# xandercai/JSPSR

Measured on AMD Instinct MI355X. Metric: Mpixels/sec fwd+bwd, JSPSR x8 on 512^2 DEM tiles, higher is better.
Workload: dtype bf16; 1 GPU; jspsr_r8_img_msk (image+mask guided, 43.87M params), 8 x 512x512 tiles per GPU, train step (fwd + L1/L2/Sobel loss + bwd + grad all-reduce + AdamW); storage policy: bf16 activations / gradients / MFMA operands, fp32 accumulation, BatchNorm statistics, master weights and optimizer, and the generator head (affinity logits + offsets) kept as fp32 planes; tiles_per_gpu=8, tile=512, global_tiles=8, parallelism=dp1, step_mode=eager

## Files before the change

### include/jspsr_hip.h

```cpp
#ifndef JSPSR_HIP_H
#define JSPSR_HIP_H

#include <stddef.h>
#include <stdint.h>

#ifdef __cplusplus
extern "C" {
#endif

#define JSPSR_OK 0
#define JSPSR_EINVAL (-1)
#define JSPSR_EALIGN (-2)

typedef void* jspsr_stream_t;

int jspsr_abi_version(void);
long long jspsr_launch_count(const char* what);
int jspsr_conv_dynamic_queue(int on);
const char* jspsr_last_error(void);

int jspsr_prop_forward_f32(const float* dem, const float* weight, const float* offset,
                           int offset_channels, const float* wk, const float* b0, float scale,
                           float* out, int B, int H, int W, jspsr_stream_t stream);

size_t jspsr_prop_backward_workspace_bytes(int B, int H, int W);

int jspsr_prop_backward_f32(const float* grad_out, const float* dem, const float* weight,
                            const float* offset, int offset_channels, const float* wk,
                            float* grad_weight, float* grad_offset, float* grad_wk,
                            float* grad_b0, void* workspace, int B, int H, int W,
                            jspsr_stream_t stream);

int jspsr_prop_backward_fold_f32(const void* workspace, int B, int H, int W, float* grad_wk, float* grad_b0,
                                 jspsr_stream_t stream);

int jspsr_prop_step_forward_f32(const float* dem, const float* weight, const float* offset, int offset_channels,
                                const float* wk, const float* b0, float scale, int normalize, float* out,
                                int B, int H, int W, jspsr_stream_t stream);
size_t jspsr_prop_step_backward_workspace_bytes(int B, int H, int W);
int jspsr_prop_step_backward_f32(const float* grad_out, const float* dem, const float* weight, const float* offset,
                                 int offset_channels, const float* wk, float scale, int normalize, int accumulate,
// ... 46 lines not shown
int jspsr_conv_head1_backward(int dtype, const float* dy, const void* x, int x_cstride, int x_coff, int C, const float* w,
                              void* dx, int dx_cstride, int dx_coff, float* dw, float* db, void* workspace, int B, int H,
                              int W, jspsr_stream_t stream);

#define JSPSR_F32 0
#define JSPSR_BF16 1

int jspsr_pack_weight(int dtype, const float* w, void* packed, int O, int I, int KH, int KW,
                      int mode, int c_pad, jspsr_stream_t stream);

typedef struct jspsr_pack_desc {
  const float* w;
  void* out;
  long long start;
  long long total;
  int O, I, KH, KW;
  int mode;
  int c_pad;
  int dtype;
  int reserved;
} jspsr_pack_desc;
int jspsr_pack_chunk(void);
int jspsr_pack_weights_multi(const jspsr_pack_desc* descs, int n, long long total_blocks, jspsr_stream_t stream);

int jspsr_conv2d_stats_rows(int B, int OH, int OW);
int jspsr_conv2d_in_affine_ok(int dtype, int Cin, int KH, int KW, int stride);
int jspsr_conv2d_forward(int dtype, const void* in, const void* wpack, const float* bias, void* out,
                         int B, int IH, int IW, int Cin, int in_cstride, int in_coff, int Cout,
                         int out_cstride, int out_coff, int KH, int KW, int stride, int pad, int relu,
                         float* stats, const float* scale, const void* addend, int add_cstride,
                         const float* in_affine, int in_relu, jspsr_stream_t stream);
int jspsr_conv2d_forward_scaled(int dtype, const void* in, const void* wpack, const float* bias, void* out,
                                int B, int IH, int IW, int Cin, int in_cstride, int in_coff, int Cout,
                                int out_cstride, int out_coff, int KH, int KW, int stride, int pad, int relu,
                                float* stats, const float* scale, const void* addend, int add_cstride,
                                const float* in_scale, int in_scale_bstride, jspsr_stream_t stream);

int jspsr_conv2d_dgrad_reduce_ok(int dtype, int B, int IH, int IW, int Cg, int Cin, int KH, int KW, int stride, int pad);
int jspsr_conv2d_dgrad(int dtype, const void* gout, const void* wpack_t, const float* bias, void* gin,
                       int B, int OH, int OW, int Cg, int g_cstride, int g_coff, int IH, int IW,
                       int Cin, int in_cstride, int in_coff, int KH, int KW, int stride, int pad,
                       int relu, const void* addend, int add_cstride, const float* scale,
                       const void* red_x, int red_cstride, const float* red_par, float* red_out, jspsr_stream_t stream);

size_t jspsr_conv2d_wgrad_workspace_bytes(int dtype, int B, int OH, int OW, int Cg, int Cx, int KH, int KW);
int jspsr_conv2d_wgrad_x_affine_ok(int dtype, int B, int OH, int OW, int Cg, int Cx, int KH, int KW, int stride, int pad);
// ... 176 lines not shown
```

### jspsr_amd/_lib.py

```python
from __future__ import annotations

import ctypes
import os
import subprocess
import threading

_HERE = os.path.dirname(os.path.abspath(__file__))
SO_PATH = os.environ.get("JSPSR_LAB_LIB") or os.path.join(_HERE, "lib", "libjspsr_hip.so")
CSRC = os.path.join(_HERE, "csrc")
ABI_VERSION = 25

_lock = threading.Lock()
_lib = None

c_p = ctypes.c_void_p
c_i = ctypes.c_int
c_f = ctypes.c_float
c_ll = ctypes.c_longlong

SIGNATURES = {
    "jspsr_abi_version": (c_i, []),
    "jspsr_launch_count": (c_ll, [ctypes.c_char_p]),
    "jspsr_conv_dynamic_queue": (c_i, [c_i]),
    "jspsr_last_error": (ctypes.c_char_p, []),
    "jspsr_prop_forward_f32": (c_i, [c_p, c_p, c_p, c_i, c_p, c_p, c_f, c_p, c_i, c_i, c_i, c_p]),
    "jspsr_prop_backward_workspace_bytes": (ctypes.c_size_t, [c_i, c_i, c_i]),
    "jspsr_prop_backward_f32": (c_i, [c_p] * 4 + [c_i] + [c_p] * 6 + [c_i, c_i, c_i, c_p]),
    "jspsr_prop_backward_fold_f32": (c_i, [c_p, c_i, c_i, c_i, c_p, c_p, c_p]),
    "jspsr_prop_step_forward_f32": (c_i, [c_p, c_p, c_p, c_i, c_p, c_p, c_f, c_i, c_p, c_i, c_i, c_i, c_p]),
    "jspsr_prop_step_backward_workspace_bytes": (ctypes.c_size_t, [c_i, c_i, c_i]),
    "jspsr_prop_step_backward_f32": (c_i, [c_p] * 4 + [c_i, c_p, c_f, c_i, c_i] + [c_p] * 6 + [c_i, c_i, c_i, c_p]),
    "jspsr_prop_head_forward": (c_i, [c_i, c_p, c_p, c_p, c_p, c_f, c_p, c_i, c_i, c_i, c_p]),
    "jspsr_prop_head_backward_workspace_bytes": (ctypes.c_size_t, [c_i, c_i, c_i]),
    "jspsr_prop_head_backward": (c_i, [c_i] + [c_p] * 8 + [c_i, c_i, c_i, c_p]),
    "jspsr_prop_logits_forward_f32": (c_i, [c_p, c_p, c_p, c_p, c_f, c_p, c_i, c_i, c_i, c_p]),
    "jspsr_prop_logits_backward_f32": (c_i, [c_p] * 8 + [c_i, c_i, c_i, c_p]),
    "jspsr_head_ok": (c_i, [c_i] * 5),
    "jspsr_head_forward": (c_i, [c_i, c_p, c_i, c_i, c_i, c_p, c_p, c_p, c_i, c_i, c_i, c_p]),
    "jspsr_head_backward_workspace_bytes": (ctypes.c_size_t, [c_i, c_i, c_i]),
    "jspsr_head_backward": (c_i, [c_i, c_p, c_p, c_i, c_p, c_i, c_i, c_p, c_p, c_p, c_i, c_i, c_i, c_p]),
    "jspsr_conv_head1_forward": (c_i, [c_i, c_p, c_i, c_i, c_i, c_p, c_p, c_p, c_i, c_i, c_i, c_p]),
    "jspsr_conv_head1_workspace_bytes": (ctypes.c_size_t, [c_i, c_i, c_i, c_i]),
    "jspsr_conv_head1_backward": (c_i, [c_i, c_p, c_p, c_i, c_i, c_i, c_p, c_p, c_i, c_i, c_p, c_p, c_p, c_i, c_i, c_i, c_p]),
    "jspsr_pack_weight": (c_i, [c_i, c_p, c_p] + [c_i] * 6 + [c_p]),
    "jspsr_pack_chunk": (c_i, []),
    "jspsr_pack_weights_multi": (c_i, [c_p, c_i, c_ll, c_p]),
    "jspsr_conv2d_stats_rows": (c_i, [c_i, c_i, c_i]),
    "jspsr_conv2d_in_affine_ok": (c_i, [c_i] * 5),
    "jspsr_conv2d_forward": (c_i, [c_i] + [c_p] * 4 + [c_i] * 14 + [c_p, c_p, c_p, c_i, c_p, c_i, c_p]),
    "jspsr_conv2d_forward_scaled": (c_i, [c_i] + [c_p] * 4 + [c_i] * 14 + [c_p, c_p, c_p, c_i, c_p, c_i, c_p]),
    "jspsr_bn_fold": (c_i, [c_p, c_p, c_p, c_p, c_f, c_f, c_i, c_p, c_p, c_p]),
    "jspsr_conv2d_dgrad_reduce_ok": (c_i, [c_i] * 10),
    "jspsr_conv2d_dgrad": (c_i, [c_i] + [c_p] * 4 + [c_i] * 16 + [c_p, c_i, c_p, c_p, c_i, c_p, c_p, c_p]),
    "jspsr_conv2d_wgrad_workspace_bytes": (ctypes.c_size_t, [c_i] * 8),
    "jspsr_conv2d_wgrad_x_affine_ok": (c_i, [c_i] * 10),
    "jspsr_conv2d_wgrad": (c_i, [c_i, c_p, c_i, c_i, c_i, c_p, c_i, c_i, c_i, c_p] + [c_i] * 12 + [c_p, c_i, c_p, c_p]),
    "jspsr_conv2d_wgrad_scaled": (c_i, [c_i, c_p, c_i, c_i, c_i, c_p, c_i, c_i, c_i, c_p] + [c_i] * 12 + [c_p, c_i, c_p, c_p]),
    "jspsr_reduce_workspace_bytes": (ctypes.c_size_t, [c_i, c_i, c_i]),
    "jspsr_bn_forward": (c_i, [c_i, c_p, c_i, c_i, c_p, c_i, c_i, c_p, c_i, c_i, c_p, c_p, c_p, c_p, c_f, c_f, c_i,
                               c_i, c_f, c_p, c_p, c_ll, c_i, c_p, c_i, c_p, c_p, c_p, c_p, c_p]),
    "jspsr_bn_mask_bytes": (ctypes.c_size_t, [c_i, c_ll, c_i]),
    "jspsr_bn_reduce_params": (c_i, [c_p, c_p, c_p, c_p, c_i, c_p, c_p]),
    "jspsr_bn_backward": (c_i, [c_i, c_p, c_i, c_i, c_p, c_i, c_i, c_p, c_i, c_i, c_p, c_p, c_p, c_p, c_i, c_i, c_f,
                                c_p, c_p, c_p, c_p, c_i, c_ll, c_i, c_p, c_p, c_i, c_p, c_p]),
    "jspsr_act_backward": (c_i, [c_i, c_p, c_i, c_i, c_p, c_i, c_i, c_p, c_i, c_p, c_ll, c_i, c_p, c_p]),
    "jspsr_gate_pool": (c_i, [c_i, c_p, c_i, c_ll, c_i, c_p, c_p, c_p, c_p, c_p]),
    "jspsr_gate_scale": (c_i, [c_i, c_p, c_p, c_p, c_i, c_ll, c_i, c_p]),
    "jspsr_gate_backward_reduce": (c_i, [c_i, c_p, c_p, c_p, c_i, c_ll, c_i, c_p, c_p]),
    "jspsr_gate_backward_apply": (c_i, [c_i, c_p, c_p, c_p, c_p, c_p, c_p, c_i, c_ll, c_i, c_p]),
# ... 108 lines not shown
```

### jspsr_amd/csrc/conv.hip

```cpp
#include "conv_igemm.h"

#include <cstdlib>
#include <type_traits>

namespace {

using namespace jspsr;

constexpr int NT = 256;
constexpr int NCH = 8;
template <typename T> struct Elem;
template <> struct Elem<float> { static constexpr int EPC = 4; };
template <> struct Elem<__bf16> { static constexpr int EPC = 8; };

template <typename T> struct Mma;
template <> struct Mma<float> {
  static constexpr int BLK = 32, ROWP = 144, NE = 16, SUB = NCH / 2, SUBB = 32;
  using acc_t = f32x16;
  static __device__ __forceinline__ int frag_row(int lane) { return lane & 31; }
  static __device__ __forceinline__ int frag_chunk(int lane) { return lane >> 5; }
  static __device__ __forceinline__ int acc_row(int lane, int e) { return (e & 3) + 8 * (e >> 2) + 4 * (lane >> 5); }
  static __device__ __forceinline__ int acc_col(int lane) { return lane & 31; }
};
template <> struct Mma<__bf16> {
// ... 1042 lines not shown
    const int mid = (lo + hi + 1) >> 1;
    if (descs[mid].start <= b) lo = mid; else hi = mid - 1;
  }
  const jspsr_pack_desc d = descs[lo];
  const long long l0 = (b - d.start) * PACK_CHUNK;
  const float* __restrict__ w = d.w;
#pragma unroll
  for (int k = 0; k < PACK_CHUNK / 256; ++k) {
    const long long l = l0 + k * 256 + threadIdx.x;
    if (l >= d.total) break;
    const int c = (int)(l % d.c_pad);
    long long r = l / d.c_pad;
    const int kx = (int)(r % d.KW); r /= d.KW;
    const int ky = (int)(r % d.KH); r /= d.KH;
    const int nn = (int)r;
    float v = 0.f;
    if (d.mode == 0) { if (c < d.I) v = w[(((size_t)nn * d.I + c) * d.KH + ky) * d.KW + kx]; }
    else             { if (c < d.O) v = w[(((size_t)c * d.I + nn) * d.KH + ky) * d.KW + kx]; }
    if (d.dtype == JSPSR_F32) static_cast<float*>(d.out)[l] = v;
    else static_cast<__bf16*>(d.out)[l] = (__bf16)v;
  }
}

}

extern "C" int jspsr_pack_weights_multi(const jspsr_pack_desc* descs, int n, long long total_blocks, jspsr_stream_t stream) {
  if (!descs || n <= 0 || total_blocks <= 0 || total_blocks > 0x7fffffffLL) return fail(JSPSR_EINVAL, "pack_weights_multi: bad arguments");
  hipLaunchKernelGGL(pack_weights_multi_kernel, dim3((unsigned)total_blocks), dim3(256), 0, static_cast<hipStream_t>(stream), descs, n);
  return check_launch("pack_weights_multi");
}

extern "C" int jspsr_pack_chunk(void) { return PACK_CHUNK; }

extern "C" int jspsr_pack_weight(int dtype, const float* w, void* packed, int O, int I, int KH, int KW,
                                 int mode, int c_pad, jspsr_stream_t stream) {
  if (!w || !packed || O <= 0 || I <= 0 || KH <= 0 || KW <= 0 || (mode != 0 && mode != 1))
    return fail(JSPSR_EINVAL, "pack_weight: bad arguments");
  const int C = mode == 0 ? I : O, N = mode == 0 ? O : I;
  if (c_pad < C) return fail(JSPSR_EINVAL, "pack_weight: c_pad %d < %d", c_pad, C);
  const long long total = (long long)N * KH * KW * c_pad;
  const int blocks = (int)((total + 255) / 256 < 4096 ? (total + 255) / 256 : 4096);
  hipStream_t s = static_cast<hipStream_t>(stream);
  if (dtype == JSPSR_F32)
    hipLaunchKernelGGL(pack_weight_kernel<float>, dim3(blocks), dim3(256), 0, s, w, static_cast<float*>(packed), O, I, KH, KW, mode, c_pad, total);
  else if (dtype == JSPSR_BF16)
    hipLaunchKernelGGL(pack_weight_kernel<__bf16>, dim3(blocks), dim3(256), 0, s, w, static_cast<__bf16*>(packed), O, I, KH, KW, mode, c_pad, total);
  else
    return fail(JSPSR_EINVAL, "pack_weight: bad dtype");
  return check_launch("pack_weight");
}

extern "C" int jspsr_conv2d_stats_rows(int B, int OH, int OW) {
  if (B <= 0 || OH <= 0 || OW <= 0) return 0;
  return B * ((OH + 7) / 8) * ((OW + 15) / 16);
}
// ... 128 lines not shown
```

### jspsr_amd/csrc/elementwise.hip

```cpp
#include "common.h"

#include <atomic>
#include <cstdlib>

namespace {

using namespace jspsr;

constexpr int TX = 64, TY = 4;

template <typename T> struct V;
template <> struct V<float> { static constexpr int N = 4; };
template <> struct V<__bf16> { static constexpr int N = 8; };

template <typename T, int N>
struct Pack { T v[N]; };

template <typename T>
__device__ __forceinline__ uint4 load_raw(const T* p) { return *reinterpret_cast<const uint4*>(p); }
template <typename T>
__device__ __forceinline__ void unpack(const uint4& raw, float (&f)[V<T>::N]) {
  if constexpr (sizeof(T) == 4) {
    f[0] = __uint_as_float(raw.x); f[1] = __uint_as_float(raw.y); f[2] = __uint_as_float(raw.z); f[3] = __uint_as_float(raw.w);
  } else {
// ... 686 lines not shown
                                void* mask_out, void* workspace, jspsr_stream_t stream) {
  if (int e = check_c(dtype, C, "bn_forward")) return e;
  if (!x || (!y && !affine_out) || !gamma || !beta || !save_mean || !save_invstd || !workspace || npix <= 0)
    return fail(JSPSR_EINVAL, "bn_forward: null pointer or empty tensor");
  if (res_affine && !res) return fail(JSPSR_EINVAL, "bn_forward: res_affine without a residual operand");
  if (mask_out && (!res || !relu || !y)) return fail(JSPSR_EINVAL, "bn_forward: mask_out needs an output with residual and ReLU");
  if (!training && (!running_mean || !running_var)) return fail(JSPSR_EINVAL, "bn_forward: eval mode needs running stats");
  const int vec = dtype == JSPSR_F32 ? 4 : 8;
  if (x_cs % vec || x_coff % vec || y_cs % vec || y_coff % vec || (res && (r_cs % vec || r_coff % vec)))
    return fail(JSPSR_EINVAL, "bn_forward: channel pitches/offsets must be multiples of %d", vec);
  hipStream_t s = static_cast<hipStream_t>(stream);
  float* ws = static_cast<float*>(workspace);
  float* scale = affine_out ? affine_out : ws;
  float* shift = affine_out ? affine_out + C : ws + C;
  float* partial = ws + 2 * C;
  int rows = 0;
  if (training && ext_partial) {
    if (ext_rows <= 0) return fail(JSPSR_EINVAL, "bn_forward: ext_rows must be positive");
    rows = ext_rows < 256 ? ext_rows : 256;
    if (ext_rows > 256) {
      hipLaunchKernelGGL(fold_rows_kernel, dim3(rows, (2 * C + 255) / 256), dim3(256), 0, s, ext_partial, ext_rows, 2 * C, rows, partial);
      if (int e = check_launch("bn_fold_rows")) return e;
    } else {
      (void)hipMemcpyAsync(partial, ext_partial, (size_t)ext_rows * 2 * C * sizeof(float), hipMemcpyDeviceToDevice, s);
    }
  } else if (training) {
    const RedGeom g = make_red(npix, 1, C, vec);
    rows = g.chunks;
    DISPATCH(dtype, hipLaunchKernelGGL(bn_stats_kernel<T>, red_grid(g, vec), dim3(TX, TY), 0, s,
                                       static_cast<const T*>(x), x_cs, x_coff, g, partial));
    if (int e = check_launch("bn_stats")) return e;
  }
  hipLaunchKernelGGL(bn_finalize_kernel, dim3((C + 3) / 4), dim3(256), 0, s, partial, rows, C, npix, gamma, beta,
                     running_mean, running_var, momentum, eps, training, save_mean, save_invstd, scale, shift);
  if (int e = check_launch("bn_finalize")) return e;
  if (!y) return JSPSR_OK;
  const RedGeom ga = make_red(npix, 1, C, vec);
#define BN_APPLY(R, M) DISPATCH(dtype, hipLaunchKernelGGL((bn_apply_kernel<T, R, M>), red_grid(ga, vec), dim3(TX, TY), 0, s,       \
                                     static_cast<const T*>(x), x_cs, x_coff, static_cast<const T*>(res), r_cs, r_coff,        \
                                     static_cast<T*>(y), y_cs, y_coff, scale, shift, res_affine, res_scale, relu,             \
                                     static_cast<unsigned char*>(mask_out), ga))
  if (mask_out) { BN_APPLY(true, true); } else if (res) { BN_APPLY(true, false); } else { BN_APPLY(false, false); }
#undef BN_APPLY
  return check_launch("bn_apply");
}

__global__ void bn_reduce_params_kernel(const float* __restrict__ gamma, const float* __restrict__ beta, const float* __restrict__ mean,
// ... 511 lines not shown
```

### jspsr_amd/csrc/wgrad.hip

```cpp
#include "conv_igemm.h"

#include <type_traits>

namespace {

using namespace jspsr;

constexpr int NT = 256;
using s16x4 = __attribute__((ext_vector_type(4))) short;

struct WgradGeom {
  int B, OH, OW;
  int Cg, g_cs, g_coff;
  int IH, IW;
  int Cx, x_cs, x_coff;
  int KH, KW, stride, pad;
  int Ktot;
  int m_per_split;
  long long M;
};

template <typename T> struct WT;
template <> struct WT<float> { static constexpr int EPC = 4, BKM = 32; };
template <> struct WT<__bf16> { static constexpr int EPC = 8, BKM = 64; };
// ... 502 lines not shown
      }
    red[zl][ex] = s;
    __syncthreads();
    if (zl == 0 && idx < total) {
      float t[4] = {0.f, 0.f, 0.f, 0.f};
#pragma unroll
      for (int q = 0; q < 8; ++q) {
        const float4 v = red[q][ex];
        t[0] += v.x; t[1] += v.y; t[2] += v.z; t[3] += v.w;
      }
#pragma unroll
      for (int j = 0; j < 4; ++j) {
        const long long i = idx + j;
        const int r = (int)(i / Ktot), k = (int)(i % Ktot);
        const int tap = k / Cx, c = k % Cx;
        if (c < C) {
          const size_t dst = ((size_t)r * C + c) * (KH * KW) + tap;
          dW[dst] = accumulate ? dW[dst] + t[j] : t[j];
        }
      }
    }
    __syncthreads();
  }
}

struct Plan {
  int bmc, splits, m_per_split;
};

template <typename T>
Plan make_plan(long long M, int Cg, int Ktot) {
  Plan p;
  p.bmc = Cg > 64 ? 128 : (Cg > 32 ? 64 : 32);
  const int BKM = WT<T>::BKM;
  const long long tiles = (long long)((Cg + p.bmc - 1) / p.bmc) * ((Ktot + 127) / 128);
  long long splits = (768 + tiles - 1) / tiles;
  const long long max_splits = (M + 4 * BKM - 1) / (4 * BKM);
  if (splits > max_splits) splits = max_splits;
  if (splits < 1) splits = 1;
  long long per = (M + splits - 1) / splits;
  per = (per + BKM - 1) / BKM * BKM;
  p.m_per_split = (int)per;
  p.splits = (int)((M + per - 1) / per);
  return p;
}

// ... 19 lines not shown
    const PatchPlan pp = make_patch_plan<T>(g.B, g.OH, g.OW, g.Cg, g.Cx);
    const long long img_g = (long long)g.OH * g.OW * g.g_cs * (long long)sizeof(T);
    const long long img_x = (long long)g.IH * g.IW * g.x_cs * (long long)sizeof(T);
    if (pp.ok && img_g < 0xF0000000LL && img_x < 0xF0000000LL) {
      PatchGeom q{};
      q.B = g.B; q.H = g.OH; q.W = g.OW;
      q.Cg = g.Cg; q.g_cs = g.g_cs; q.g_coff = g.g_coff;
      q.Cx = g.Cx; q.x_cs = g.x_cs; q.x_coff = g.x_coff;
      q.Ktot = g.Ktot; q.strips_x = g.OW / WP<T>::U;
      q.rows_per_blk = pp.rows_per_blk; q.row_blks = pp.row_blks;
      q.pairs_g = (g.Cg + 63) / 64; q.pairs_x = (g.Cx + 63) / 64;
      q.x_affine = x_affine; q.x_relu = x_relu; q.x_bstride = x_bstride; q.x_scale_only = x_scale_only;
      const long long nblk = (long long)pp.units * q.pairs_g * q.pairs_x;
      if (x_affine && x_scale_only)
        hipLaunchKernelGGL((wgrad_patch_kernel<T, 2>), dim3((unsigned)nblk), dim3(NT), 0, s, static_cast<const T*>(G),
                           static_cast<const T*>(X), ws, q);
      else if (x_affine)
        hipLaunchKernelGGL((wgrad_patch_kernel<T, 1>), dim3((unsigned)nblk), dim3(NT), 0, s, static_cast<const T*>(G),
                           static_cast<const T*>(X), ws, q);
      else
        hipLaunchKernelGGL((wgrad_patch_kernel<T, 0>), dim3((unsigned)nblk), dim3(NT), 0, s, static_cast<const T*>(G),
                           static_cast<const T*>(X), ws, q);
      if (int e = check_launch("conv2d_wgrad_patch")) return e;
      const long long total = (long long)R * g.Ktot;
      const int blocks = (int)((total + 127) / 128 < 4096 ? (total + 127) / 128 : 4096);
      hipLaunchKernelGGL(wgrad_reduce_kernel, dim3(blocks), dim3(256), 0, s, ws, dW, R, C, g.KH, g.KW, g.Cg, g.Cx,
                         pp.units, accumulate);
      return check_launch("conv2d_wgrad_reduce");
    }
  }
  if (x_affine) return fail(JSPSR_EINVAL, "conv2d_wgrad: x_affine needs the nine-tap kernel (3x3, stride 1, pad 1): ask jspsr_conv2d_wgrad_x_affine_ok first");
  const Plan p = make_plan<T>(g.M, g.Cg, g.Ktot);
  g.m_per_split = p.m_per_split;
  const long long g_slice = (long long)p.m_per_split * g.g_cs * (long long)sizeof(T);
  const long long imgs = p.m_per_split / ((long long)g.OH * g.OW) + 2;
  const long long x_span = imgs * g.IH * g.IW * (long long)g.x_cs * (long long)sizeof(T);
  if (g_slice >= 0xF0000000LL || (x_span >= 0xF0000000LL && (long long)g.B * g.IH * g.IW * g.x_cs * (long long)sizeof(T) >= 0xF0000000LL))
    return fail(JSPSR_EINVAL, "conv2d_wgrad: tensor slice exceeds the 32-bit offset range of one launch");
  int e;
  if (p.bmc == 128) e = launch_w<T, 128, 2, 2>(G, X, ws, g, p.splits, s);
  else if (p.bmc == 64) e = launch_w<T, 64, 2, 2>(G, X, ws, g, p.splits, s);
  else e = launch_w<T, 32, 1, 4>(G, X, ws, g, p.splits, s);
  if (e) return e;
  const long long total = (long long)R * g.Ktot;
  const int blocks = (int)((total + 127) / 128 < 4096 ? (total + 127) / 128 : 4096);
  hipLaunchKernelGGL(wgrad_reduce_kernel, dim3(blocks), dim3(256), 0, s, ws, dW, R, C, g.KH, g.KW, g.Cg, g.Cx,
                     p.splits, accumulate);
  return check_launch("conv2d_wgrad_reduce");
}

}

extern "C" size_t jspsr_conv2d_wgrad_workspace_bytes(int dtype, int B, int OH, int OW, int Cg, int Cx, int KH, int KW) {
  if (B <= 0 || OH <= 0 || OW <= 0 || Cg <= 0 || Cx <= 0 || KH <= 0 || KW <= 0) return 0;
  const long long M = (long long)B * OH * OW;
  const int Ktot = KH * KW * Cx;
  const Plan p = dtype == JSPSR_BF16 ? make_plan<__bf16>(M, Cg, Ktot) : make_plan<float>(M, Cg, Ktot);
  size_t splits = (size_t)p.splits;
  if (KH == 3 && KW == 3) {
    const PatchPlan pp = dtype == JSPSR_BF16 ? make_patch_plan<__bf16>(B, OH, OW, Cg, Cx) : make_patch_plan<float>(B, OH, OW, Cg, Cx);
    if (pp.ok && (size_t)pp.units > splits) splits = (size_t)pp.units;
  }
  return splits * Cg * Ktot * sizeof(float);
}

static int conv2d_wgrad_impl(int dtype, const void* G, int Cg, int g_cstride, int g_coff, const void* X, int Cx,
                             int x_cstride, int x_coff, float* dW, int R, int C, int B, int OH, int OW,
                             int IH, int IW, int KH, int KW, int stride, int pad, int accumulate,
                             const float* x_affine, int x_relu, int x_bstride, int x_scale_only, void* workspace,
                             jspsr_stream_t stream) {
  if (dtype != JSPSR_F32 && dtype != JSPSR_BF16) return fail(JSPSR_EINVAL, "conv2d_wgrad: bad dtype");
  if (x_affine && !aligned16(x_affine)) return fail(JSPSR_EALIGN, "conv2d_wgrad: x_affine must be 16-byte aligned");
  if (!G || !X || !dW || !workspace) return fail(JSPSR_EINVAL, "conv2d_wgrad: null pointer");
// ... 44 lines not shown
```

### jspsr_amd/graph.py

```python
from __future__ import annotations

import torch

from . import ops


class GraphedStep:

    def __init__(self, model, reducer, optimizer, criterion, inputs, target, warmup: int = 3):
        if reducer.world != 1:
            raise RuntimeError("GraphedStep: single-process steps only (a captured step holds no collective)")
        if not model.training:
            raise RuntimeError("GraphedStep captures a TRAINING step: call model.train() first")
        self.model, self.reducer, self.opt, self.criterion = model, reducer, optimizer, criterion
        self.inputs = [t.detach().clone() for t in inputs]
        self.target = target.detach().clone()
        optimizer.enable_device_hyper()
        if hasattr(criterion, "reset"):
            criterion.reset()
        import gc
        gc.collect()
        side = torch.cuda.Stream()
        side.wait_stream(torch.cuda.current_stream())
        with torch.cuda.stream(side):
            for _ in range(warmup):
                self._body()
            if hasattr(criterion, "reset"):
                criterion.reset()
        torch.cuda.current_stream().wait_stream(side)
        torch.cuda.synchronize()
        self.warmup_steps = warmup
        steps_before = optimizer.steps
        self.graph = torch.cuda.CUDAGraph()
        with torch.cuda.graph(self.graph, stream=side):
            self.loss = self._body()
        optimizer.steps = steps_before
        self.replays = 0

    def _body(self):
        self.reducer.zero_grad()
        loss = self.criterion(self.model(*self.inputs), self.target)["Total"]
        loss.backward()
        self.reducer.finish()
        self.opt.step()
        return loss

    def __call__(self, inputs=None, target=None):
        if inputs is not None:
            for dst, src in zip(self.inputs, inputs):
                dst.copy_(src, non_blocking=True)
        if target is not None:
            self.target.copy_(target, non_blocking=True)
        self.opt.steps += 1
        self.opt.upload_hyper()
        self.graph.replay()
        ops.invalidate_packed_weights()
        self.replays += 1
        return self.loss
```

### jspsr_amd/kernels.py

```python
from __future__ import annotations

import torch

from . import _lib

F32, BF16 = 0, 1


def _dt(t: torch.Tensor) -> int:
    if t.dtype == torch.float32:
        return F32
    if t.dtype == torch.bfloat16:
        return BF16
    raise TypeError(f"unsupported dtype {t.dtype}")


def epc(dtype: torch.dtype) -> int:
    return 4 if dtype == torch.float32 else 8


def _stream() -> int:
    return torch.cuda.current_stream().cuda_stream


# ... 9 lines not shown
        return False
    B, H, W, C = t.shape
    p = t.stride(2)
    if p < C or (H > 1 and t.stride(1) != W * p) or (B > 1 and t.stride(0) != H * W * p) or W == 1:
        return False
    return t.data_ptr() % 16 == 0 and (p * t.element_size()) % 16 == 0


def pitch(t: torch.Tensor) -> int:
    return t.shape[3] if t.is_contiguous() else t.stride(2)


def nhwc(t: torch.Tensor) -> torch.Tensor:
    return t if (t.is_contiguous() or is_slice(t)) else t.contiguous()


def _chk_s(t: torch.Tensor, name: str):
    if not t.is_cuda:
        raise RuntimeError(f"{name}: jspsr_amd kernels run on the GPU only (no CPU fallback)")
    if not (t.is_contiguous() or is_slice(t)):
        raise ValueError(f"{name}: expected a dense NHWC tensor or a channel slice of one")


def pack_weight(w: torch.Tensor, mode: int, c_pad: int, dtype: torch.dtype) -> torch.Tensor:
    _chk(w, "pack_weight")
    O, I, KH, KW = w.shape
    n = O if mode == 0 else I
    out = torch.empty((n, KH, KW, c_pad), dtype=dtype, device=w.device)
    lib = _lib.load()
    _lib.check(lib.jspsr_pack_weight(_dt(out), w.data_ptr(), out.data_ptr(), O, I, KH, KW, mode, c_pad, _stream()),
               "jspsr_pack_weight")
    return out


def fused_input_ok(dtype, B, OH, OW, Cin, Cout, KH, KW, stride, pad) -> bool:
    lib = _lib.load()
    dt = F32 if dtype == torch.float32 else BF16
    return bool(lib.jspsr_conv2d_in_affine_ok(dt, Cin, KH, KW, stride)) and \
        bool(lib.jspsr_conv2d_wgrad_x_affine_ok(dt, B, OH, OW, Cout, Cin, KH, KW, stride, pad))


def _chk_scale(t, B, C, name):
    if t.dtype != torch.float32 or not t.is_cuda or not t.is_contiguous() or tuple(t.shape) != (B, C):
        raise ValueError(f"{name}: expected a contiguous fp32 ({B}, {C}) tensor on the GPU, got {tuple(t.shape)} {t.dtype}")


def in_scale_ok(dtype, Cin, KH, KW, stride) -> bool:
    return bool(_lib.load().jspsr_conv2d_in_affine_ok(F32 if dtype == torch.float32 else BF16, Cin, KH, KW, stride))


def x_scale_ok(dtype, B, OH, OW, Cout, Cin, KH, KW, stride, pad) -> bool:
# ... 316 lines not shown
```

### jspsr_amd/ops.py

```python
from __future__ import annotations

import collections
import os
import weakref

import torch

from . import _lib
from . import kernels as K


def _stream() -> int:
    return torch.cuda.current_stream().cuda_stream


def _need_gpu(*ts):
    for t in ts:
        if not t.is_cuda:
            raise RuntimeError("jspsr_amd ops run on the GPU only (got a CPU tensor); there is no CPU fallback")
        if t.dtype != torch.float32:
            raise TypeError(f"expected float32, got {t.dtype}")


def prop_forward_raw(dem, weight, offset, w, b, scale, out):
# ... 393 lines not shown
        ws = torch.empty(max(lib.jspsr_prop_backward_workspace_bytes(B, H, W), 16), dtype=torch.uint8, device=dem.device)
        _lib.check(lib.jspsr_prop_logits_backward_f32(grad_out.data_ptr(), dem.data_ptr(), head.data_ptr(), w.data_ptr(),
                                                      ghead.data_ptr(), gw.data_ptr(), gb.data_ptr(), ws.data_ptr(), B, H, W,
                                                      _stream()), "jspsr_prop_logits_backward_f32")
        return None, ghead, gw, gb, None


def propagate_logits(dem, head, w, b, scale: float = 1.0):
    if dem.requires_grad:
        raise RuntimeError("propagate_logits: dem must be detached (no gradient with respect to the DEM is produced)")
    return _PropagateLogits.apply(dem, head, w, b, scale)




_weights_epoch = 0


def invalidate_packed_weights():
    global _weights_epoch
    _weights_epoch += 1


repack_after_step = os.environ.get("JSPSR_REPACK_ALL", "0") != "0"
_pack_registry = {}
_pack_table = None


def _packed(param, w, mode, c_pad, dtype):
    if not isinstance(param, torch.nn.Parameter):
        return K.pack_weight(w, mode, c_pad, dtype)
    cache = param.__dict__.setdefault("_jspsr_packs", {})
    key = (mode, c_pad, dtype, w.data_ptr())
    hit = cache.get(key)
    stamp = (param._version, _weights_epoch)
    if hit is not None and hit[1] == stamp:
        return hit[0]
    if len(cache) > 8:
        cache.clear()
    packed = K.pack_weight(w, mode, c_pad, dtype)
    cache[key] = (packed, stamp)
    if id(param) not in _pack_registry:
        _pack_registry[id(param)] = weakref.ref(param, lambda _, k=id(param): _pack_registry.pop(k, None))
    return packed


def repack_all():
    global _pack_table
    import numpy as np
    entries = []
    for ref in list(_pack_registry.values()):
        p = ref()
        if p is None or not p.is_cuda:
            continue
        for (mode, c_pad, dtype, ptr), (packed, _) in p.__dict__.get("_jspsr_packs", {}).items():
            if ptr == p.data_ptr() and p.dim() == 4 and p.is_contiguous():
                entries.append((p, mode, c_pad, dtype, packed))
    if not entries:
        return 0
    sig = tuple((p.data_ptr(), packed.data_ptr(), mode, c_pad) for p, mode, c_pad, _, packed in entries)
    if _pack_table is None or _pack_table[0] != sig:
        desc = np.zeros(len(entries), dtype=np.dtype([("w", "<u8"), ("out", "<u8"), ("start", "<i8"), ("total", "<i8"),
                                                      ("O", "<i4"), ("I", "<i4"), ("KH", "<i4"), ("KW", "<i4"), ("mode", "<i4"),
                                                      ("c_pad", "<i4"), ("dtype", "<i4"), ("reserved", "<i4")]))
        start, chunk = 0, _lib.load().jspsr_pack_chunk()
        for i, (p, mode, c_pad, dtype, packed) in enumerate(entries):
            O, I, KH, KW = p.shape
            total = packed.numel()
            desc[i] = (p.data_ptr(), packed.data_ptr(), start, total, O, I, KH, KW, mode, c_pad, K._dt(packed), 0)
            start += (total + chunk - 1) // chunk
        table = torch.from_numpy(desc.view(np.uint8).copy()).to(entries[0][0].device)
        _pack_table = (sig, table, start)
    _, table, grand = _pack_table
    _lib.check(_lib.load().jspsr_pack_weights_multi(table.data_ptr(), len(entries), grand, _stream()), "jspsr_pack_weights_multi")
    for p, mode, c_pad, dtype, packed in entries:
        p.__dict__["_jspsr_packs"][(mode, c_pad, dtype, p.data_ptr())] = (packed, (p._version, _weights_epoch))
    return len(entries)


def pad_channels(x: torch.Tensor, mult: int) -> torch.Tensor:
    c = x.shape[-1]
    p = (-c) % mult
    return x if p == 0 else torch.nn.functional.pad(x, (0, p))


def _wgrad_into(param, G, X, R, C, KH, KW, stride, pad, **kw):
    gbuf = param.grad if param is not None and getattr(param, "_jspsr_direct_grad", False) else None
    if (gbuf is not None and gbuf.dtype == torch.float32 and gbuf.is_contiguous() and gbuf.is_cuda
            and tuple(gbuf.shape) == (R, C, KH, KW)):
        K.conv2d_wgrad(G, X, R, C, KH, KW, stride, pad, out=gbuf, accumulate=True, **kw)
        ready = getattr(param, "_jspsr_grad_ready", None)
        if ready is not None:
            ready(param)
        return None
    return K.conv2d_wgrad(G, X, R, C, KH, KW, stride, pad, **kw)


_aux_streams = {}
_marks = {}
# ... 539 lines not shown
```

Baseline: 36.69 Mpixel/s.

## Add LDS-tiled weight repack, run-based wgrad reduce, and drop BN partial copy

Adds a tiled weight-pack kernel that stages weight tiles in LDS before transposing into packed layout, enables repack-all by default, and repacks into existing packed buffers in place. Adds a new wgrad split-reduction kernel that sums split slabs with float4 loads and writes contiguous runs per output row. Replaces a device-to-device copy of BN partial statistics with pointer aliasing. These target memory traffic and launch overhead in the per-step weight repack and wgrad reduction, at the cost of more complex descriptor planning and a capture-time restriction.

```diff
diff --git a/include/jspsr_hip.h b/include/jspsr_hip.h
--- a/include/jspsr_hip.h
+++ b/include/jspsr_hip.h
@@ -17,6 +17,7 @@
 int jspsr_abi_version(void);
 long long jspsr_launch_count(const char* what);
 int jspsr_conv_dynamic_queue(int on);
+int jspsr_wgrad_reduce_form(int form);
 const char* jspsr_last_error(void);
 
 int jspsr_prop_forward_f32(const float* dem, const float* weight, const float* offset,
@@ -109,6 +110,22 @@
 } jspsr_pack_desc;
 int jspsr_pack_chunk(void);
 int jspsr_pack_weights_multi(const jspsr_pack_desc* descs, int n, long long total_blocks, jspsr_stream_t stream);
+
+typedef struct jspsr_pack_tile {
+  const float* w;
+  void* out;
+  long long start;
+  long long total;
+  int O, I, KH, KW;
+  int mode;
+  int c_pad;
+  int dtype;
+  int ti, to;
+  int ninner;
+  int reserved[2];
+} jspsr_pack_tile;
+int jspsr_pack_lds_floats(void);
+int jspsr_pack_weights_tiled(const jspsr_pack_tile* tiles, int n, long long total_blocks, jspsr_stream_t stream);
 
 int jspsr_conv2d_stats_rows(int B, int OH, int OW);
 int jspsr_conv2d_in_affine_ok(int dtype, int Cin, int KH, int KW, int stride);
diff --git a/jspsr_amd/_lib.py b/jspsr_amd/_lib.py
--- a/jspsr_amd/_lib.py
+++ b/jspsr_amd/_lib.py
@@ -22,6 +22,7 @@
     "jspsr_abi_version": (c_i, []),
     "jspsr_launch_count": (c_ll, [ctypes.c_char_p]),
     "jspsr_conv_dynamic_queue": (c_i, [c_i]),
+    "jspsr_wgrad_reduce_form": (c_i, [c_i]),
     "jspsr_last_error": (ctypes.c_char_p, []),
     "jspsr_prop_forward_f32": (c_i, [c_p, c_p, c_p, c_i, c_p, c_p, c_f, c_p, c_i, c_i, c_i, c_p]),
     "jspsr_prop_backward_workspace_bytes": (ctypes.c_size_t, [c_i, c_i, c_i]),
@@ -45,6 +46,8 @@
     "jspsr_pack_weight": (c_i, [c_i, c_p, c_p] + [c_i] * 6 + [c_p]),
     "jspsr_pack_chunk": (c_i, []),
     "jspsr_pack_weights_multi": (c_i, [c_p, c_i, c_ll, c_p]),
+    "jspsr_pack_lds_floats": (c_i, []),
+    "jspsr_pack_weights_tiled": (c_i, [c_p, c_i, c_ll, c_p]),
     "jspsr_conv2d_stats_rows": (c_i, [c_i, c_i, c_i]),
     "jspsr_conv2d_in_affine_ok": (c_i, [c_i] * 5),
     "jspsr_conv2d_forward": (c_i, [c_i] + [c_p] * 4 + [c_i] * 14 + [c_p, c_p, c_p, c_i, c_p, c_i, c_p]),
diff --git a/jspsr_amd/csrc/conv.hip b/jspsr_amd/csrc/conv.hip
--- a/jspsr_amd/csrc/conv.hip
+++ b/jspsr_amd/csrc/conv.hip
@@ -1088,6 +1088,74 @@
   }
 }
 
+constexpr int PACK_LDS = 9280;
+
+template <typename T>
+__device__ __forceinline__ void pack_tile(const jspsr_pack_tile& d, int u, float* lds) {
+  const int taps = d.KH * d.KW;
+  const float* __restrict__ w = d.w;
+  T* __restrict__ out = static_cast<T*>(d.out);
+  const int lane = threadIdx.x & 63, wave = threadIdx.x >> 6;
+  if (d.ti <= 0 || d.to <= 0 || d.ninner <= 0 || taps <= 0 || d.c_pad < (d.mode == 0 ? d.I : d.O)) return;
+  const int outer = d.mode == 0 ? (d.O + d.to - 1) / d.to : (d.I + d.ti - 1) / d.ti;
+  if (u < 0 || (long long)u >= (long long)outer * d.ninner) return;
+  if (d.mode == 0) {
+    const int ot = u / d.ninner, ch = u - ot * d.ninner;
+    const int o0 = ot * d.to, i0 = ch * d.ti;
+    const int tov = min(d.to, d.O - o0), tiv = min(d.ti, d.I - i0);
+    if (tov <= 0 || tiv <= 0 || (tov > 1 && tiv != d.I)) return;
+    const int n = tov * tiv * taps;
+    if (n > PACK_LDS) return;
+    const float* __restrict__ src = w + ((size_t)o0 * d.I + i0) * taps;
+    for (int e = threadIdx.x; e < n; e += 256) lds[e] = src[e];
+    __syncthreads();
+    const int cw = ch == d.ninner - 1 ? d.c_pad - i0 : tiv;
+    for (int rt = wave; rt < tov * taps; rt += 4) {
+      const int ol = rt / taps, tap = rt - ol * taps;
+      T* __restrict__ dst = out + ((size_t)(o0 + ol) * taps + tap) * d.c_pad + i0;
+      const float* s = lds + ol * tiv * taps + tap;
+      for (int c = lane; c < cw; c += 64) dst[c] = (T)(c < tiv ? s[c * taps] : 0.f);
+    }
+  } else {
+    const int it = u / d.ninner, ot = u - it * d.ninner;
+    const int i0 = it * d.ti, o0 = ot * d.to;
+    const int tiv = min(d.ti, d.I - i0);
+    const int tow = min(d.to, d.c_pad - o0);
+    const int tov = max(0, min(d.to, d.O - o0));
+    if (tiv <= 0 || tow <= 0) return;
+    const int run = tiv * taps, pitch = run | 1;
+    if ((long long)tov * pitch > PACK_LDS) return;
+    for (int ol = wave; ol < tov; ol += 4) {
+      const float* __restrict__ src = w + ((size_t)(o0 + ol) * d.I + i0) * taps;
+      for (int e = lane; e < run; e += 64) lds[ol * pitch + e] = src[e];
+    }
+    __syncthreads();
+    for (int rt = wave; rt < run; rt += 4) {
+      T* __restrict__ dst = out + ((size_t)i0 * taps + rt) * d.c_pad + o0;
+      for (int ol = lane; ol < tow; ol += 64) dst[ol] = (T)(ol < tov ? lds[ol * pitch + rt] : 0.f);
+    }
+  }
+}
+
+__global__ __launch_bounds__(256) void pack_weights_tiled_kernel(const jspsr_pack_tile* __restrict__ descs, int n) {
+  __shared__ float lds[PACK_LDS];
+  const long long b = blockIdx.x;
+  int mine = 0;
+  for (int i = threadIdx.x; i < n; i += 256) mine += descs[i].start <= b ? 1 : 0;
+  __shared__ int cnt;
+  if (threadIdx.x == 0) cnt = 0;
+  __syncthreads();
+  if (mine) atomicAdd(&cnt, mine);
+  __syncthreads();
+  const int k = cnt - 1;
+  if (k < 0) return;
+  const jspsr_pack_tile d = descs[k];
+  const long long u = b - d.start;
+  if (u < 0 || u > 0x7fffffffLL) return;
+  if (d.dtype == JSPSR_F32) pack_tile<float>(d, (int)u, lds);
+  else pack_tile<__bf16>(d, (int)u, lds);
+}
+
 }
 
 extern "C" int jspsr_pack_weights_multi(const jspsr_pack_desc* descs, int n, long long total_blocks, jspsr_stream_t stream) {
@@ -1097,6 +1165,14 @@
 }
 
 extern "C" int jspsr_pack_chunk(void) { return PACK_CHUNK; }
+
+extern "C" int jspsr_pack_weights_tiled(const jspsr_pack_tile* tiles, int n, long long total_blocks, jspsr_stream_t stream) {
+  if (!tiles || n <= 0 || total_blocks <= 0 || total_blocks > 0x7fffffffLL) return fail(JSPSR_EINVAL, "pack_weights_tiled: bad arguments");
+  hipLaunchKernelGGL(pack_weights_tiled_kernel, dim3((unsigned)total_blocks), dim3(256), 0, static_cast<hipStream_t>(stream), tiles, n);
+  return check_launch("pack_weights_multi");
+}
+
+extern "C" int jspsr_pack_lds_floats(void) { return PACK_LDS; }
 
 extern "C" int jspsr_pack_weight(int dtype, const float* w, void* packed, int O, int I, int KH, int KW,
                                  int mode, int c_pad, jspsr_stream_t stream) {
diff --git a/jspsr_amd/csrc/elementwise.hip b/jspsr_amd/csrc/elementwise.hip
--- a/jspsr_amd/csrc/elementwise.hip
+++ b/jspsr_amd/csrc/elementwise.hip
@@ -732,7 +732,7 @@
       hipLaunchKernelGGL(fold_rows_kernel, dim3(rows, (2 * C + 255) / 256), dim3(256), 0, s, ext_partial, ext_rows, 2 * C, rows, partial);
       if (int e = check_launch("bn_fold_rows")) return e;
     } else {
-      (void)hipMemcpyAsync(partial, ext_partial, (size_t)ext_rows * 2 * C * sizeof(float), hipMemcpyDeviceToDevice, s);
+      partial = const_cast<float*>(ext_partial);
     }
   } else if (training) {
     const RedGeom g = make_red(npix, 1, C, vec);
diff --git a/jspsr_amd/csrc/wgrad.hip b/jspsr_amd/csrc/wgrad.hip
--- a/jspsr_amd/csrc/wgrad.hip
+++ b/jspsr_amd/csrc/wgrad.hip
@@ -1,5 +1,6 @@
 #include "conv_igemm.h"
 
+#include <atomic>
 #include <type_traits>
 
 namespace {
@@ -548,6 +549,103 @@
     }
     __syncthreads();
   }
+}
+
+constexpr int REDUCE_PARK = 1152;
+
+__host__ __device__ inline int reduce_cb(int taps) {
+  const int cb = (REDUCE_PARK / taps) & ~3;
+  return cb > 128 ? 128 : cb;
+}
+
+__global__ __launch_bounds__(256) void wgrad_reduce_runs_kernel(const float* __restrict__ ws, float* __restrict__ dW, int R,
+                                                               int C, int taps, int Cg, int Cx, int splits, int accumulate,
+                                                               int CB, int nCB) {
+  __shared__ float4 red[2][8][32];
+  __shared__ float park[REDUCE_PARK];
+  const int Ktot = taps * Cx;
+  const size_t slab = (size_t)Cg * Ktot;
+  const int r = blockIdx.x / nCB, c0 = (blockIdx.x - r * nCB) * CB;
+  if (r >= R || c0 >= C) return;
+  const int cbv = min(CB, C - c0);
+  const int cb4 = (cbv + 3) >> 2;
+  const int items = taps * cb4;
+  const int ex = threadIdx.x & 31, zl = threadIdx.x >> 5;
+  const float* __restrict__ row = ws + (size_t)r * Ktot + c0;
+  for (int base = 0, pass = 0; base < items; base += 32, ++pass) {
+    const int item = base + ex;
+    const int tap = item / cb4, g4 = item - tap * cb4;
+    float4 s = make_float4(0.f, 0.f, 0.f, 0.f);
+    if (item < items) {
+      const float* __restrict__ src = row + tap * Cx + 4 * g4;
+      int z = zl;
+      for (; z + 24 < splits; z += 32) {
+        const float4 v0 = *reinterpret_cast<const float4*>(src + z * slab);
+        const float4 v1 = *reinterpret_cast<const float4*>(src + (z + 8) * slab);
+        const float4 v2 = *reinterpret_cast<const float4*>(src + (z + 16) * slab);
+        const float4 v3 = *reinterpret_cast<const float4*>(src + (z + 24) * slab);
+        s.x += v0.x; s.y += v0.y; s.z += v0.z; s.w += v0.w;
+        s.x += v1.x; s.y += v1.y; s.z += v1.z; s.w += v1.w;
+        s.x += v2.x; s.y += v2.y; s.z += v2.z; s.w += v2.w;
+        s.x += v3.x; s.y += v3.y; s.z += v3.z; s.w += v3.w;
+      }
+      for (; z < splits; z += 8) {
+        const float4 v = *reinterpret_cast<const float4*>(src + z * slab);
+        s.x += v.x; s.y += v.y; s.z += v.z; s.w += v.w;
+      }
+    }
+    red[pass & 1][zl][ex] = s;
+    __syncthreads();
+    if (threadIdx.x < 128) {
+      const int e = threadIdx.x, it = base + (e >> 2), j = e & 3;
+      const int tp = it / cb4, c = 4 * (it - tp * cb4) + j;
+      if (it < items && c < cbv) {
+        const float* f = reinterpret_cast<const float*>(&red[pass & 1][0][0]);
+        float t = 0.f;
+#pragma unroll
+        for (int q = 0; q < 8; ++q) t += f[q * 128 + e];
+        park[c * taps + tp] = t;
+      }
+    }
+  }
+  __syncthreads();
+  float* __restrict__ dst = dW + ((size_t)r * C + c0) * taps;
+  const int n = cbv * taps;
+  constexpr int U = 5;
+  for (int base = 0; base < n; base += 256 * U) {
+    float old[U];
+#pragma unroll
+    for (int k = 0; k < U; ++k) {
+      const int e = base + k * 256 + threadIdx.x;
+      old[k] = (accumulate && e < n) ? dst[e] : 0.f;
+    }
+#pragma unroll
+    for (int k = 0; k < U; ++k) {
+      const int e = base + k * 256 + threadIdx.x;
+      if (e < n) dst[e] = accumulate ? old[k] + park[e] : park[e];
+    }
+  }
+}
+
+std::atomic<int> g_reduce_form{-1};
+
+int launch_reduce(const float* ws, float* dW, int R, int C, const WgradGeom& g, int splits, int accumulate, hipStream_t s) {
+  const int taps = g.KH * g.KW;
+  int CB = reduce_cb(taps);
+  while (CB > 16 && (long long)R * ((C + CB - 1) / CB) < 2048) CB = (CB / 2) & ~3;
+  if (g_reduce_form.load(std::memory_order_relaxed) != 0 && CB > 0) {
+    const int nCB = (C + CB - 1) / CB;
+    const long long blocks = (long long)R * nCB;
+    if (blocks <= 0x7fffffffLL) {
+      hipLaunchKernelGGL(wgrad_reduce_runs_kernel, dim3((unsigned)blocks), dim3(256), 0, s, ws, dW, R, C, taps, g.Cg, g.Cx, splits,
+                         accumulate, CB, nCB);
+      return check_launch("conv2d_wgrad_reduce");
+    }
+  }
+  const long long total = (long long)R * g.Ktot;
+  const int blocks = (int)((total + 127) / 128 < 4096 ? (total + 127) / 128 : 4096);
+  hipLaunchKernelGGL(wgrad_reduce_kernel, dim3(blocks), dim3(256), 0, s, ws, dW, R, C, g.KH, g.KW, g.Cg, g.Cx, splits, accumulate);
+  return check_launch("conv2d_wgrad_reduce");
 }
 
 struct Plan {
@@ -613,11 +711,7 @@
         hipLaunchKernelGGL((wgrad_patch_kernel<T, 0>), dim3((unsigned)nblk), dim3(NT), 0, s, static_cast<const T*>(G),
                            static_cast<const T*>(X), ws, q);
       if (int e = check_launch("conv2d_wgrad_patch")) return e;
-      const long long total = (long long)R * g.Ktot;
-      const int blocks = (int)((total + 127) / 128 < 4096 ? (total + 127) / 128 : 4096);
-      hipLaunchKernelGGL(wgrad_reduce_kernel, dim3(blocks), dim3(256), 0, s, ws, dW, R, C, g.KH, g.KW, g.Cg, g.Cx,
-                         pp.units, accumulate);
-      return check_launch("conv2d_wgrad_reduce");
+      return launch_reduce(ws, dW, R, C, g, pp.units, accumulate, s);
     }
   }
   if (x_affine) return fail(JSPSR_EINVAL, "conv2d_wgrad: x_affine needs the nine-tap kernel (3x3, stride 1, pad 1): ask jspsr_conv2d_wgrad_x_affine_ok first");
@@ -633,13 +727,13 @@
   else if (p.bmc == 64) e = launch_w<T, 64, 2, 2>(G, X, ws, g, p.splits, s);
   else e = launch_w<T, 32, 1, 4>(G, X, ws, g, p.splits, s);
   if (e) return e;
-  const long long total = (long long)R * g.Ktot;
-  const int blocks = (int)((total + 127) / 128 < 4096 ? (total + 127) / 128 : 4096);
-  hipLaunchKernelGGL(wgrad_reduce_kernel, dim3(blocks), dim3(256), 0, s, ws, dW, R, C, g.KH, g.KW, g.Cg, g.Cx,
-                     p.splits, accumulate);
-  return check_launch("conv2d_wgrad_reduce");
-}
-
+  return launch_reduce(ws, dW, R, C, g, p.splits, accumulate, s);
+}
+
+}
+
+extern "C" int jspsr_wgrad_reduce_form(int form) {
+  return g_reduce_form.exchange(form < 0 ? -1 : (form ? 1 : 0), std::memory_order_relaxed);
 }
 
 extern "C" size_t jspsr_conv2d_wgrad_workspace_bytes(int dtype, int B, int OH, int OW, int Cg, int Cx, int KH, int KW) {
diff --git a/jspsr_amd/graph.py b/jspsr_amd/graph.py
--- a/jspsr_amd/graph.py
+++ b/jspsr_amd/graph.py
@@ -35,6 +35,8 @@
         with torch.cuda.graph(self.graph, stream=side):
             self.loss = self._body()
         optimizer.steps = steps_before
+        self._packs = ops.packed_entries()
+        self._pack_table = ops._pack_table if ops.repack_after_step else None
         self.replays = 0
 
     def _body(self):
@@ -55,5 +57,8 @@
         self.opt.upload_hyper()
         self.graph.replay()
         ops.invalidate_packed_weights()
+        if self._pack_table is not None:
+            for p, e in self._pack_table[3]:
+                e[1] = (p._version, ops._weights_epoch)
         self.replays += 1
         return self.loss
diff --git a/jspsr_amd/kernels.py b/jspsr_amd/kernels.py
--- a/jspsr_amd/kernels.py
+++ b/jspsr_amd/kernels.py
@@ -55,11 +55,14 @@
         raise ValueError(f"{name}: expected a dense NHWC tensor or a channel slice of one")
 
 
-def pack_weight(w: torch.Tensor, mode: int, c_pad: int, dtype: torch.dtype) -> torch.Tensor:
+def pack_weight(w: torch.Tensor, mode: int, c_pad: int, dtype: torch.dtype, out: torch.Tensor = None) -> torch.Tensor:
     _chk(w, "pack_weight")
     O, I, KH, KW = w.shape
     n = O if mode == 0 else I
-    out = torch.empty((n, KH, KW, c_pad), dtype=dtype, device=w.device)
+    if out is None:
+        out = torch.empty((n, KH, KW, c_pad), dtype=dtype, device=w.device)
+    elif tuple(out.shape) != (n, KH, KW, c_pad) or out.dtype != dtype or out.device != w.device or not out.is_contiguous():
+        raise ValueError(f"pack_weight: out must be a contiguous {(n, KH, KW, c_pad)} {dtype} tensor on {w.device}")
     lib = _lib.load()
     _lib.check(lib.jspsr_pack_weight(_dt(out), w.data_ptr(), out.data_ptr(), O, I, KH, KW, mode, c_pad, _stream()),
                "jspsr_pack_weight")
diff --git a/jspsr_amd/ops.py b/jspsr_amd/ops.py
--- a/jspsr_amd/ops.py
+++ b/jspsr_amd/ops.py
@@ -439,7 +439,7 @@
     _weights_epoch += 1
 
 
-repack_after_step = os.environ.get("JSPSR_REPACK_ALL", "0") != "0"
+repack_after_step = os.environ.get("JSPSR_REPACK_ALL", "1") != "0"
 _pack_registry = {}
 _pack_table = None
 
@@ -451,47 +451,59 @@
     key = (mode, c_pad, dtype, w.data_ptr())
     hit = cache.get(key)
     stamp = (param._version, _weights_epoch)
-    if hit is not None and hit[1] == stamp:
+    if hit is not None:
+        hit[2] = True
+        if hit[1] != stamp:
+            K.pack_weight(w, mode, c_pad, dtype, out=hit[0])
+            hit[1] = stamp
         return hit[0]
     if len(cache) > 8:
         cache.clear()
     packed = K.pack_weight(w, mode, c_pad, dtype)
-    cache[key] = (packed, stamp)
+    cache[key] = [packed, stamp, True]
     if id(param) not in _pack_registry:
         _pack_registry[id(param)] = weakref.ref(param, lambda _, k=id(param): _pack_registry.pop(k, None))
     return packed
 
 
+def packed_entries():
+    out = []
+    for ref in list(_pack_registry.values()):
+        p = ref()
+        if p is not None:
+            out.extend((p, e) for e in p.__dict__.get("_jspsr_packs", {}).values())
+    return out
+
+
 def repack_all():
     global _pack_table
     import numpy as np
+    from . import packplan
     entries = []
     for ref in list(_pack_registry.values()):
         p = ref()
         if p is None or not p.is_cuda:
             continue
-        for (mode, c_pad, dtype, ptr), (packed, _) in p.__dict__.get("_jspsr_packs", {}).items():
-            if ptr == p.data_ptr() and p.dim() == 4 and p.is_contiguous():
-                entries.append((p, mode, c_pad, dtype, packed))
+        for (mode, c_pad, dtype, ptr), e in p.__dict__.get("_jspsr_packs", {}).items():
+            if e[2] and ptr == p.data_ptr() and p.dim() == 4 and p.is_contiguous():
+                entries.append((p, mode, c_pad, e))
     if not entries:
         return 0
-    sig = tuple((p.data_ptr(), packed.data_ptr(), mode, c_pad) for p, mode, c_pad, _, packed in entries)
+    sig = tuple((p.data_ptr(), e[0].data_ptr(), mode, c_pad, tuple(p.shape)) for p, mode, c_pad, e in entries)
     if _pack_table is None or _pack_table[0] != sig:
-        desc = np.zeros(len(entries), dtype=np.dtype([("w", "<u8"), ("out", "<u8"), ("start", "<i8"), ("total", "<i8"),
-                                                      ("O", "<i4"), ("I", "<i4"), ("KH", "<i4"), ("KW", "<i4"), ("mode", "<i4"),
-                                                      ("c_pad", "<i4"), ("dtype", "<i4"), ("reserved", "<i4")]))
-        start, chunk = 0, _lib.load().jspsr_pack_chunk()
-        for i, (p, mode, c_pad, dtype, packed) in enumerate(entries):
-            O, I, KH, KW = p.shape
-            total = packed.numel()
-            desc[i] = (p.data_ptr(), packed.data_ptr(), start, total, O, I, KH, KW, mode, c_pad, K._dt(packed), 0)
-            start += (total + chunk - 1) // chunk
+        if torch.cuda.is_current_stream_capturing():
+            raise RuntimeError("repack_all: under stream capture the descriptor table of the preceding eager steps must "
+                               "match the packed weights in use (building one is a host-to-device copy, illegal in a "
+                               "capture): run at least one eager step with the same model and dtype first")
+        desc, tiles = packplan.table([(p.data_ptr(), e[0].data_ptr(), *p.shape, mode, c_pad, K._dt(e[0]))
+                                      for p, mode, c_pad, e in entries])
         table = torch.from_numpy(desc.view(np.uint8).copy()).to(entries[0][0].device)
-        _pack_table = (sig, table, start)
-    _, table, grand = _pack_table
-    _lib.check(_lib.load().jspsr_pack_weights_multi(table.data_ptr(), len(entries), grand, _stream()), "jspsr_pack_weights_multi")
-    for p, mode, c_pad, dtype, packed in entries:
-        p.__dict__["_jspsr_packs"][(mode, c_pad, dtype, p.data_ptr())] = (packed, (p._version, _weights_epoch))
+        _pack_table = (sig, table, tiles, [(p, e) for p, _, _, e in entries])
+    _, table, tiles, _ = _pack_table
+    _lib.check(_lib.load().jspsr_pack_weights_tiled(table.data_ptr(), len(entries), tiles, _stream()), "jspsr_pack_weights_tiled")
+    for p, mode, c_pad, e in entries:
+        e[1] = (p._version, _weights_epoch)
+        e[2] = False
     return len(entries)
 
 
diff --git a/jspsr_amd/packplan.py b/jspsr_amd/packplan.py
--- /dev/null
+++ b/jspsr_amd/packplan.py
@@ -0,0 +1,66 @@
+from __future__ import annotations
+
+import numpy as np
+
+LDS_FLOATS = 9280
+TILE0_FLOATS = 4608
+RUN1_FLOATS = 144
+TO1 = 64
+
+DESC_DTYPE = np.dtype([("w", "<u8"), ("out", "<u8"), ("start", "<i8"), ("total", "<i8"),
+                       ("O", "<i4"), ("I", "<i4"), ("KH", "<i4"), ("KW", "<i4"), ("mode", "<i4"), ("c_pad", "<i4"),
+                       ("dtype", "<i4"), ("ti", "<i4"), ("to", "<i4"), ("ninner", "<i4"), ("reserved", "<i4", (2,))])
+assert DESC_DTYPE.itemsize == 80
+
+
+def plan(O: int, I: int, KH: int, KW: int, mode: int, c_pad: int):
+    taps = KH * KW
+    if min(O, I, KH, KW) <= 0 or mode not in (0, 1) or c_pad < (I if mode == 0 else O):
+        raise ValueError(f"pack plan: bad geometry {(O, I, KH, KW, mode, c_pad)}")
+    if mode == 0:
+        if I * taps <= TILE0_FLOATS:
+            ti, to = I, max(1, min(O, TILE0_FLOATS // (I * taps)))
+        else:
+            ti, to = TILE0_FLOATS // taps // 8 * 8, 1
+            if ti <= 0:
+                raise ValueError(f"pack plan: a {KH}x{KW} kernel does not fit the staging buffer")
+        ninner = -(-I // ti)
+        return ti, to, ninner, -(-O // to) * ninner
+    ti = max(1, min(I, RUN1_FLOATS // taps))
+    to = min(TO1, LDS_FLOATS // ((ti * taps) | 1))
+    if to <= 0:
+        raise ValueError(f"pack plan: a {KH}x{KW} kernel does not fit the staging buffer")
+    ninner = -(-c_pad // to)
+    return ti, to, ninner, -(-I // ti) * ninner
+
+
+def table(entries):
+    desc = np.zeros(len(entries), dtype=DESC_DTYPE)
+    start = 0
+    for k, (w, out, O, I, KH, KW, mode, c_pad, dt) in enumerate(entries):
+        ti, to, ninner, tiles = plan(O, I, KH, KW, mode, c_pad)
+        rows = O if mode == 0 else I
+        desc[k] = (w, out, start, rows * KH * KW * c_pad, O, I, KH, KW, mode, c_pad, dt, ti, to, ninner, (0, 0))
+        start += tiles
+    return desc, start
+
+
+def tile_writes(d, u: int) -> np.ndarray:
+    O, I, taps, c_pad = int(d["O"]), int(d["I"]), int(d["KH"]) * int(d["KW"]), int(d["c_pad"])
+    ti, to, ninner = int(d["ti"]), int(d["to"]), int(d["ninner"])
+    if int(d["mode"]) == 0:
+        ot, ch = divmod(u, ninner)
+        o0, i0 = ot * to, ch * ti
+        tov, tiv = min(to, O - o0), min(ti, I - i0)
+        if tov <= 0 or tiv <= 0 or (tov > 1 and tiv != I) or tov * tiv * taps > LDS_FLOATS:
+            return np.zeros(0, dtype=np.int64)
+        cw = c_pad - i0 if ch == ninner - 1 else tiv
+        rows = (o0 * taps + np.arange(tov * taps, dtype=np.int64)) * c_pad + i0
+        return (rows[:, None] + np.arange(cw, dtype=np.int64)[None, :]).reshape(-1)
+    it, ot = divmod(u, ninner)
+    i0, o0 = it * ti, ot * to
+    tiv, tow, tov = min(ti, I - i0), min(to, c_pad - o0), max(0, min(to, O - o0))
+    if tiv <= 0 or tow <= 0 or tov * ((tiv * taps) | 1) > LDS_FLOATS:
+        return np.zeros(0, dtype=np.int64)
+    rows = (i0 * taps + np.arange(tiv * taps, dtype=np.int64)) * c_pad + o0
+    return (rows[:, None] + np.arange(tow, dtype=np.int64)[None, :]).reshape(-1)
```

Measured after the change: 37.03 Mpixel/s, median of 6. Within noise of the previous version (+0.9%).
